# antonbaumann/MIMO-Unet

Measured on AMD Instinct MI355X. Metric: train images/sec at 256x256, S=2, fbc=30, higher is better.
Workload: dtype f32 (split into 16-bit hi/lo pairs on the MFMA; weight gradient: activation as one fp16 value); 1 GPU; cfg3: SEN12TP-shape synthetic 2->1 ch, 256x256, S=2, fbc=30, laplace_nll, batch 32 global; global_batch=32, per_gpu_batch=32, scaling=strong, labels=U[0,1) (SURVEY 8d); same batch every step, parallelism=dp1, world_size=1, weak_per_gpu_batch=32, strong_global_batch=32, optimizer=adam(lr=1e-3) fused, inputs=resident in HBM

## Files before the change

mimo_unet_amd/csrc/elementwise.hip:

```cpp
#include <hip/hip_ext.h>

#include <algorithm>
#include <cstdlib>

#include "elementwise.h"
#include "philox.h"

namespace mimo {

struct PQ {
  int q;
  int ql, pl;
  int QB, PPI;
  int p, pstep;
  bool active;
};

template <int T = 256>
__device__ __forceinline__ PQ pixquad(int Cv, bool xcd_bands = false) {
  PQ r;
  r.QB = Cv < T ? Cv : T;
  r.PPI = T / r.QB;
  r.ql = threadIdx.x % r.QB;
  r.pl = threadIdx.x / r.QB;
  r.q = blockIdx.y * r.QB + r.ql;
  r.active = r.pl < r.PPI && r.q < Cv;
  int bx = blockIdx.x;
  if (xcd_bands && (gridDim.x & 7) == 0) bx = (bx & 7) * (gridDim.x >> 3) + (bx >> 3);
  r.p = bx * r.PPI + r.pl;
  r.pstep = gridDim.x * r.PPI;
  return r;
}

constexpr int kBlocksBnRelu = 1536, kBlocksBnBwd = 1792, kBlocksUpBwd = 16384, kBlocksPoolBwd = 8192;
constexpr int kBnReduceThreads = 1024, kBlocksBnReduce = kBlocksBnBwd / 4;
static dim3 pq_grid(int Cv, int64_t P, int max_blocks = kEwMaxBlocks, int T = 256) {
  const int QB = Cv < T ? Cv : T;
  const int PPI = T / QB;
  int64_t gx = ceil_div64(P, PPI);
  if (gx > max_blocks) gx = max_blocks;
  if (gx < 1) gx = 1;
  return dim3((unsigned)gx, (unsigned)ceil_div(Cv, QB));
}

__device__ __forceinline__ float4 ld4(const float* p) { return *reinterpret_cast<const float4*>(p); }
__device__ __forceinline__ void st4(float* p, float4 v) { *reinterpret_cast<float4*>(p) = v; }
typedef __bf16 bf16x4_st __attribute__((ext_vector_type(4)));
typedef _Float16 f16x4_st __attribute__((ext_vector_type(4)));
__device__ __forceinline__ float4 ld4(const __bf16* p) {
  const bf16x4_st v = *reinterpret_cast<const bf16x4_st*>(p);
  return make_float4((float)v[0], (float)v[1], (float)v[2], (float)v[3]);
}
__device__ __forceinline__ void st4(__bf16* p, float4 v) {
  bf16x4_st r;
  r[0] = (__bf16)v.x;
  r[1] = (__bf16)v.y;
  r[2] = (__bf16)v.z;
  r[3] = (__bf16)v.w;
  *reinterpret_cast<bf16x4_st*>(p) = r;
}
__device__ __forceinline__ float4 ld4(const _Float16* p) {
  const f16x4_st v = *reinterpret_cast<const f16x4_st*>(p);
  return make_float4((float)v[0], (float)v[1], (float)v[2], (float)v[3]);
}
__device__ __forceinline__ void st4(_Float16* p, float4 v) {
  f16x4_st r;
  r[0] = (_Float16)v.x;
  r[1] = (_Float16)v.y;
  r[2] = (_Float16)v.z;
  r[3] = (_Float16)v.w;
  *reinterpret_cast<f16x4_st*>(p) = r;
}
#define MIMO_ST_DISPATCH(DT, T, ...) \
  switch (DT) {                      \
    case ST_BF16: {                  \
      typedef __bf16 T;              \
      __VA_ARGS__;                   \
    } break;                         \
    case ST_F16: {                   \
      typedef _Float16 T;            \
      __VA_ARGS__;                   \
    } break;                         \
    default: {                       \
      typedef float T;               \
      __VA_ARGS__;                   \
    } break;                         \
  }
#define MIMO_ST_DISPATCH2(DTZ, DTA, TZ, TA, ...) \
  if ((DTZ) == ST_F32) {                         \
    typedef float TZ;                            \
    MIMO_ST_DISPATCH(DTA, TA, __VA_ARGS__)       \
  } else if ((DTA) == ST_BF16) {                 \
    typedef __bf16 TZ;                           \
    typedef __bf16 TA;                           \
    __VA_ARGS__;                                 \
  } else {                                       \
    typedef _Float16 TZ;                         \
    typedef _Float16 TA;                         \
    __VA_ARGS__;                                 \
  }

__device__ __forceinline__ float4 f4add(float4 a, float4 b) { return make_float4(a.x + b.x, a.y + b.y, a.z + b.z, a.w + b.w); }
__device__ __forceinline__ float4 f4zero() { return make_float4(0.f, 0.f, 0.f, 0.f); }
__device__ __forceinline__ float4 f4max(float4 a, float4 b) {
  return make_float4(fmaxf(a.x, b.x), fmaxf(a.y, b.y), fmaxf(a.z, b.z), fmaxf(a.w, b.w));
}

__device__ __forceinline__ float4 quad_block_sum(float4 v, const PQ& t, float4* red) {
  __syncthreads();
  red[threadIdx.x] = t.active ? v : f4zero();
  __syncthreads();
  float4 s = f4zero();
  if (t.PPI <= 32) {
    if (t.pl == 0)
      for (int j = 0; j < t.PPI; ++j) s = f4add(s, red[j * t.QB + t.ql]);
    return s;
  }
  const bool lead = t.pl < 16 && t.pl < t.PPI;
  if (lead)
    for (int j = t.pl; j < t.PPI; j += 16) s = f4add(s, red[j * t.QB + t.ql]);
  __syncthreads();
  if (lead) red[threadIdx.x] = s;
  __syncthreads();
  s = f4zero();
  if (t.pl == 0)
    for (int j = 0; j < 16 && j < t.PPI; ++j) s = f4add(s, red[j * t.QB + t.ql]);
  return s;
}

template <typename T>
__device__ __forceinline__ float4 fold_read(const T* dxpad, int ldp, int n, int y, int x, int H, int W, int ch) {
  const T* base = dxpad + (size_t)n * (H + 2) * (W + 2) * ldp + ch;
  float4 s = ld4(base + ((size_t)(y + 1) * (W + 2) + (x + 1)) * ldp);
  const bool ya = y == 1, yb = y == H - 2, xa = x == 1, xb = x == W - 2;
  if (ya | yb | xa | xb) {
    const int ry[3] = {y, -1, H}, rx[3] = {x, -1, W};
    const bool vy[3] = {true, ya, yb}, vx[3] = {true, xa, xb};
#pragma unroll
    for (int i = 0; i < 3; ++i)
#pragma unroll
      for (int j = 0; j < 3; ++j)
        if (i + j > 0 && vy[i] && vx[j]) s = f4add(s, ld4(base + ((size_t)(ry[i] + 1) * (W + 2) + (rx[j] + 1)) * ldp));
  }
  return s;
}

struct PixIter {
  int n, y, x, dn, dy, dx;
};
__device__ __forceinline__ PixIter pix_iter(int p0, int pstep, int H, int W) {
  PixIter it;
  const int HW = H * W;
  it.n = p0 / HW;
  int r = p0 - it.n * HW;
  it.y = r / W;
  it.x = r - it.y * W;
  it.dn = pstep / HW;
  r = pstep - it.dn * HW;
// ... 879 lines not shown
          for (int j = 0; j < 6; ++j) {
            const float ww = ey[e] * (j < 4 ? wx[j] : ex[j - 4]);
            v.x += ww * g[j].x;
            v.y += ww * g[j].y;
            v.z += ww * g[j].z;
            v.w += ww * g[j].w;
          }
        }
        if (ex[e] != 0.f) {
          float4 g[4];
#pragma unroll
          for (int k = 0; k < 4; ++k) g[k] = ld4(base + ((size_t)(cy[k] + 1) * (W + 2) + prx[e]) * ldp);
#pragma unroll
          for (int k = 0; k < 4; ++k) {
            const float ww = wy[k] * ex[e];
            v.x += ww * g[k].x;
            v.y += ww * g[k].y;
            v.z += ww * g[k].z;
            v.w += ww * g[k].w;
          }
        }
      }
    }
    return v;
}

template <typename T>
__global__ void up_bwd_kernel(const T* __restrict__ dxpad, int ldp, int choff, T* __restrict__ da, int ldda,
                              int N, int H, int W, int h, int w, int padT, int padL, int Cv, int accumulate) {
  const PQ t = pixquad(Cv, true);
  if (!t.active) return;
  const int P = N * h * w;
  PixIter it = pix_iter(t.p, t.pstep, h, w);
  for (int p = t.p; p < P; p += t.pstep, pix_next(it, h, w)) {
    float4 v = up_bwd_pixel(dxpad, ldp, choff, t.q, it.n, it.y, it.x, H, W, h, w, padT, padL);
    T* dst = da + (size_t)p * ldda + 4 * t.q;
    if (accumulate) v = f4add(v, ld4(dst));
    st4(dst, v);
  }
}


int up_bwd_launch(const void* dxpad, int dt, int ldp, int choff, void* da, int ldda, int N, int H, int W, int h, int w,
                  int Cp, int accumulate, hipStream_t st) {
  const int Cv = Cp / 4;
  const int padT = (H - 2 * h) / 2, padL = (W - 2 * w) / 2;
  MIMO_ST_DISPATCH(dt, T, hipLaunchKernelGGL(up_bwd_kernel<T>, pq_grid(Cv, (int64_t)N * h * w, kBlocksUpBwd), dim3(256), 0, st,
                                             (const T*)dxpad, ldp, choff, (T*)da, ldda, N, H, W, h, w, padT, padL, Cv, accumulate));
  MIMO_KERNEL_CHECK();
  return MIMO_OK;
}

__device__ __forceinline__ float nll_value(int kind, float d, float lp, float eps_min, float eps_max) {
  const float sc = fminf(fmaxf(expf(lp), eps_min), eps_max);
  return kind == MIMO_LOSS_LAPLACE_NLL ? logf(sc) + fabsf(d) / sc : logf(sc) + d * d / sc;
}
__device__ __forceinline__ void nll_grad(int kind, float d, float lp, float eps_min, float eps_max, float* gmu, float* glp) {
  const float e = expf(lp);
  const float sc = fminf(fmaxf(e, eps_min), eps_max);
  if (kind == MIMO_LOSS_LAPLACE_NLL) {
    const float sgn = d > 0.f ? 1.f : (d < 0.f ? -1.f : 0.f);
    *gmu = sgn / sc;
    *glp = (1.f / sc - fabsf(d) / (sc * sc)) * e;
  } else {
    *gmu = 2.f * d / sc;
    *glp = (1.f / sc - d * d / (sc * sc)) * e;
  }
}

struct HeadLane {
  float4 w0, w1;
  float coef;
};
__device__ __forceinline__ HeadLane head_lane(const HeadGrad& h, int q, bool active) {
  HeadLane l;
  l.w0 = l.w1 = f4zero();
  l.coef = h.dloss ? h.dloss[h.s] * h.inv_count : 0.f;
  if (active) {
    const int c0 = 4 * q;
    float* a0 = reinterpret_cast<float*>(&l.w0);
    float* a1 = reinterpret_cast<float*>(&l.w1);
#pragma unroll
    for (int j = 0; j < 4; ++j) {
      a0[j] = c0 + j < h.C ? h.w[c0 + j] : 0.f;
      a1[j] = c0 + j < h.C ? h.w[h.C + c0 + j] : 0.f;
    }
  }
  return l;
}
__device__ __forceinline__ void head_dlogit(const HeadGrad& h, const HeadLane& l, int p, float* d0, float* d1) {
  const int n = p / h.HW;
  const int yx = p - n * h.HW;
  const int64_t obase = (((int64_t)n * h.S + h.s) * 2) * h.HW + yx;
  float a = h.dout ? h.dout[obase] : 0.f, b = h.dout ? h.dout[obase + h.HW] : 0.f;
  if (h.dloss) {
    const int64_t src = h.perm ? h.perm[(int64_t)h.s * h.N + n] : n;
    const float mk = h.mask ? h.mask[src * h.HW + yx] : 1.f;
    const float mu = h.out[obase], lp = h.out[obase + h.HW], y = h.label[src * h.HW + yx];
    float gm, gl;
    nll_grad(h.kind, mu - y, lp, h.eps_min, h.eps_max, &gm, &gl);
    a += l.coef * mk * gm;
    b += l.coef * mk * gl;
  }
  *d0 = a;
  *d1 = b;
}

__device__ __forceinline__ float4 relu_gate4(float4 g, float4 v, float4 sc, float4 sh) {
  g.x = fmaf(v.x, sc.x, sh.x) > 0.f ? g.x : 0.f;
  g.y = fmaf(v.y, sc.y, sh.y) > 0.f ? g.y : 0.f;
  g.z = fmaf(v.z, sc.z, sh.z) > 0.f ? g.z : 0.f;
  g.w = fmaf(v.w, sc.w, sh.w) > 0.f ? g.w : 0.f;
  return g;
}

template <typename TZ, typename TA>
__device__ __forceinline__ int pool_cell4(const GradSrc& s, const TZ* z, int ldz, int n, int cy, int cx, int H, int W, int q,
                                          float4 sc, float4 sh, bool masked, float4 m, float4 zz[4], float4 g[4]) {
  const int Hp = H / 2, Wp = W / 2, y0 = 2 * cy, x0 = 2 * cx;
  const bool win = cy < Hp && cx < Wp;
  const int valid = win ? 15 : ((1 | (x0 + 1 < W ? 2 : 0)) | (y0 + 1 < H ? (4 | (x0 + 1 < W ? 8 : 0)) : 0));
  const TZ* zs = z + (((size_t)n * H + y0) * W + x0) * ldz + 4 * q;
#pragma unroll
  for (int j = 0; j < 4; ++j) zz[j] = (valid >> j) & 1 ? ld4(zs + ((size_t)(j >> 1) * W + (j & 1)) * ldz) : f4zero();
  float4 gp = f4zero();
  if (win) gp = fold_read((const TA*)s.dxpad, s.ldp, n, cy, cx, Hp, Wp, s.choff + 4 * q);
#pragma unroll
  for (int j = 0; j < 4; ++j)
    g[j] = (s.skip && ((valid >> j) & 1)) ? fold_read((const TA*)s.skip, s.ldsk, n, y0 + (j >> 1), x0 + (j & 1), H, W, s.skoff + 4 * q)
                                           : f4zero();
  if (win) {
    auto act = [&](float v, float k, float b, float mm) { return fmaxf(fmaf(v, k, b), 0.f) * mm; };
#pragma unroll
    for (int j = 0; j < 4; ++j) {
      g[j].x = route_max(gp.x, act(zz[0].x, sc.x, sh.x, m.x), act(zz[1].x, sc.x, sh.x, m.x), act(zz[2].x, sc.x, sh.x, m.x), act(zz[3].x, sc.x, sh.x, m.x), j) + g[j].x;
      g[j].y = route_max(gp.y, act(zz[0].y, sc.y, sh.y, m.y), act(zz[1].y, sc.y, sh.y, m.y), act(zz[2].y, sc.y, sh.y, m.y), act(zz[3].y, sc.y, sh.y, m.y), j) + g[j].y;
      g[j].z = route_max(gp.z, act(zz[0].z, sc.z, sh.z, m.z), act(zz[1].z, sc.z, sh.z, m.z), act(zz[2].z, sc.z, sh.z, m.z), act(zz[3].z, sc.z, sh.z, m.z), j) + g[j].z;
      g[j].w = route_max(gp.w, act(zz[0].w, sc.w, sh.w, m.w), act(zz[1].w, sc.w, sh.w, m.w), act(zz[2].w, sc.w, sh.w, m.w), act(zz[3].w, sc.w, sh.w, m.w), j) + g[j].w;
    }
  }
#pragma unroll
  for (int j = 0; j < 4; ++j) {
    if (masked) {
      g[j].x *= m.x;
      g[j].y *= m.y;
      g[j].z *= m.z;
      g[j].w *= m.w;
    }
    g[j] = relu_gate4(g[j], zz[j], sc, sh);
  }
  return valid;
}

template <int SRC, typename TZ, typename TA>
__device__ __forceinline__ float4 relu_grad4(const GradSrc& s, const HeadLane& hl, const float* mask, int C, int p,
                                             const PixIter& it, int q, int H, int W, float4 v, float4 sc, float4 sh, float* d0,
                                             float* d1) {
  static_assert(SRC != GS_POOL, "pooled tensors: pool_cell4");
  float4 g;
  const int n = it.n;
  float4 m = make_float4(1.f, 1.f, 1.f, 1.f);
  if (mask) m = mask4(mask, n, C, 4 * q);
  if constexpr (SRC == GS_PLAIN) {
    g = ld4((const TA*)s.da + (size_t)p * s.ldda + 4 * q);
  } else if constexpr (SRC == GS_FOLD) {
    g = fold_read((const TA*)s.dxpad, s.ldp, n, it.y, it.x, H, W, 4 * q);
  } else {
    head_dlogit(s.head, hl, p, d0, d1);
    g = f4zero();
    g.x = fmaf(*d1, hl.w1.x, fmaf(*d0, hl.w0.x, g.x));
    g.y = fmaf(*d1, hl.w1.y, fmaf(*d0, hl.w0.y, g.y));
    g.z = fmaf(*d1, hl.w1.z, fmaf(*d0, hl.w0.z, g.z));
    g.w = fmaf(*d1, hl.w1.w, fmaf(*d0, hl.w0.w, g.w));
  }
  if (mask) {
    g.x *= m.x;
    g.y *= m.y;
    g.z *= m.z;
    g.w *= m.w;
  }
  return relu_gate4(g, v, sc, sh);
}

template <typename TZ, typename TA, int SRC>
__global__ __launch_bounds__(kBnReduceThreads) void bnrelu_bwd_reduce_kernel(
    const GradSrc src, const TZ* __restrict__ z, int ldz,
    const float* __restrict__ scale, const float* __restrict__ shift, const float* __restrict__ mean,
    const float* __restrict__ invstd, const float* __restrict__ mask, int C, int Cv, int N, int H, int W,
    float* __restrict__ partial) {
  __shared__ float4 red[kBnReduceThreads];
  const PQ t = pixquad<kBnReduceThreads>(Cv);
  const int Cp = 4 * Cv;
  float4 a1 = f4zero(), a2 = f4zero();
  float4 hw0 = f4zero(), hw1 = f4zero();
  float hb0 = 0.f, hb1 = 0.f;
  HeadLane hl = {};
  if constexpr (SRC == GS_HEAD) hl = head_lane(src.head, t.q, t.active);
  if (t.active) {
    const float4 sc = ld4(scale + 4 * t.q), sh = ld4(shift + 4 * t.q), mu = ld4(mean + 4 * t.q), is = ld4(invstd + 4 * t.q);
    if constexpr (SRC == GS_POOL) {
      const int Hc = (H + 1) / 2, Wc = (W + 1) / 2, P = N * Hc * Wc;
      PixIter it = pix_iter(t.p, t.pstep, Hc, Wc);
      for (int p = t.p; p < P; p += t.pstep, pix_next(it, Hc, Wc)) {
        float4 zz[4], g[4];
        const float4 m = mask ? mask4(mask, it.n, C, 4 * t.q) : make_float4(1.f, 1.f, 1.f, 1.f);
        const int valid = pool_cell4<TZ, TA>(src, z, ldz, it.n, it.y, it.x, H, W, t.q, sc, sh, mask != nullptr, m, zz, g);
#pragma unroll
        for (int j = 0; j < 4; ++j)
          if ((valid >> j) & 1) {
            a1 = f4add(a1, g[j]);
            a2.x += g[j].x * (zz[j].x - mu.x) * is.x;
            a2.y += g[j].y * (zz[j].y - mu.y) * is.y;
            a2.z += g[j].z * (zz[j].z - mu.z) * is.z;
            a2.w += g[j].w * (zz[j].w - mu.w) * is.w;
          }
      }
    } else {
      const int P = N * H * W;
      PixIter it = pix_iter(t.p, t.pstep, H, W);
      for (int p = t.p; p < P; p += t.pstep, pix_next(it, H, W)) {
        const float4 v = ld4(z + (size_t)p * ldz + 4 * t.q);
        float d0 = 0.f, d1 = 0.f;
        const float4 g = relu_grad4<SRC, TZ, TA>(src, hl, mask, C, p, it, t.q, H, W, v, sc, sh, &d0, &d1);
        a1 = f4add(a1, g);
        a2.x += g.x * (v.x - mu.x) * is.x;
        a2.y += g.y * (v.y - mu.y) * is.y;
        a2.z += g.z * (v.z - mu.z) * is.z;
        a2.w += g.w * (v.w - mu.w) * is.w;
        if constexpr (SRC == GS_HEAD) {
          const float4 av = bn_relu4(v, sc, sh);
          hw0.x = fmaf(d0, av.x, hw0.x);
          hw0.y = fmaf(d0, av.y, hw0.y);
          hw0.z = fmaf(d0, av.z, hw0.z);
          hw0.w = fmaf(d0, av.w, hw0.w);
          hw1.x = fmaf(d1, av.x, hw1.x);
          hw1.y = fmaf(d1, av.y, hw1.y);
          hw1.z = fmaf(d1, av.z, hw1.z);
          hw1.w = fmaf(d1, av.w, hw1.w);
          hb0 += d0;
          hb1 += d1;
        }
      }
    }
  }
  const float4 s1 = quad_block_sum(a1, t, red);
  const float4 s2 = quad_block_sum(a2, t, red);
  if (t.pl == 0 && t.q < Cv) {
    float* row = partial + (size_t)blockIdx.x * 2 * Cp;
    st4(row + 4 * t.q, s1);
    st4(row + Cp + 4 * t.q, s2);
  }
  if constexpr (SRC == GS_HEAD) {
    float* row = src.head.partial + (size_t)blockIdx.x * (2 * Cp + 2);
    const float4 w0 = quad_block_sum(hw0, t, red);
    const float4 w1 = quad_block_sum(hw1, t, red);
    const float4 sb = quad_block_sum(make_float4(hb0, hb1, 0.f, 0.f), t, red);
    if (t.pl == 0 && t.q < Cv) {
      st4(row + 4 * t.q, w0);
      st4(row + Cp + 4 * t.q, w1);
    }
    if (t.pl == 0 && t.q == 0) {
      row[2 * Cp] = sb.x;
      row[2 * Cp + 1] = sb.y;
    }
  }
}

static int check_grad_src(const GradSrc& src, int dta, int dtz) {
  if (src.kind < GS_PLAIN || src.kind > GS_HEAD || (src.kind >= GS_POOL && (dta != ST_F32 || dtz != ST_F32)) ||
      (src.kind == GS_HEAD && src.head.Co != 2)) {
    set_error("BatchNorm backward: gradient source %d unsupported here", src.kind);
    return MIMO_ERR_INVALID;
  }
  return MIMO_OK;
}

int bnrelu_bwd_reduce_launch(const GradSrc& src, int dta, const void* z, int dtz, int ldz,
                             const float* scale, const float* shift, const float* mean, const float* invstd,
                             const float* mask, int C, int Cp, int N, int H, int W, float* partial, int* rows,
                             hipStream_t st) {
  MIMO_TRY(check_grad_src(src, dta, dtz));
  const int Cv = Cp / 4;
  const int64_t units = src.kind == GS_POOL ? (int64_t)N * ((H + 1) / 2) * ((W + 1) / 2) : (int64_t)N * H * W;
  const dim3 grid = pq_grid(Cv, units, src.kind >= GS_POOL ? 256 : kBlocksBnReduce, kBnReduceThreads);
  *rows = grid.x;
#define REDUCE_LAUNCH(TZ, TA, SRC)                                                                                              \
  hipLaunchKernelGGL((bnrelu_bwd_reduce_kernel<TZ, TA, SRC>), grid, dim3(kBnReduceThreads), 0, st, src, (const TZ*)z, ldz, scale, \
                     shift, mean, invstd, mask, C, Cv, N, H, W, partial)
  if (src.kind == GS_POOL) {
    REDUCE_LAUNCH(float, float, GS_POOL);
  } else if (src.kind == GS_HEAD) {
    REDUCE_LAUNCH(float, float, GS_HEAD);
  } else if (src.kind == GS_PLAIN) {
    MIMO_ST_DISPATCH2(dtz, dta, TZ, TA, REDUCE_LAUNCH(TZ, TA, GS_PLAIN))
  } else {
    MIMO_ST_DISPATCH2(dtz, dta, TZ, TA, REDUCE_LAUNCH(TZ, TA, GS_FOLD))
  }
#undef REDUCE_LAUNCH
  MIMO_KERNEL_CHECK();
  return MIMO_OK;
}

__global__ __launch_bounds__(kColsumThreads) void bn_bwd_stats_kernel(const float* __restrict__ partial, int rows, int C,
                                                                      int Cp, double count, int training,
                                                                      float* __restrict__ c1, float* __restrict__ c2,
                                                                      float* __restrict__ dgamma, float* __restrict__ dbeta,
                                                                      float* __restrict__ dbias_zero, int* __restrict__ status) {
  __shared__ double red[2048];
  const int c = blockIdx.x * 64 + (threadIdx.x & 63);
  double s1, s2;
  grid_colsum2(partial, rows, (size_t)2 * Cp, c, Cp + c, c < Cp, true, red, &s1, &s2);
  if (c >= Cp || threadIdx.x >= 64) return;
  if (status && c < C && !(isfinite(s1) && isfinite(s2))) atomicOr(status, kStatusBwdStats);
  c1[c] = training ? (float)(s1 / count) : 0.f;
  c2[c] = training ? (float)(s2 / count) : 0.f;
  if (c < C) {
    if (dgamma) dgamma[c] = (float)s2;
    if (dbeta) dbeta[c] = (float)s1;
    if (dbias_zero) dbias_zero[c] = 0.f;
  }
}

int bn_bwd_stats_launch(const float* partial, int rows, int C, int Cp, int64_t count, int training, float* c1, float* c2,
                        float* dgamma, float* dbeta, float* dbias_zero, int* status, hipStream_t st) {
  hipLaunchKernelGGL(bn_bwd_stats_kernel, dim3(ceil_div(Cp, 64)), dim3(kColsumThreads), 0, st, partial, rows, C, Cp, (double)count,
                     training, c1, c2, dgamma, dbeta, dbias_zero, status);
  MIMO_KERNEL_CHECK();
  return MIMO_OK;
}

typedef __bf16 bf16x4_ew __attribute__((ext_vector_type(4)));
__device__ __forceinline__ void st_split4(float* base, size_t p, int Cp, int q, float4 r) {
  bf16x4_ew hi, lo;
  hi[0] = (__bf16)r.x;
  hi[1] = (__bf16)r.y;
  hi[2] = (__bf16)r.z;
  hi[3] = (__bf16)r.w;
  lo[0] = (__bf16)(r.x - (float)hi[0]);
  lo[1] = (__bf16)(r.y - (float)hi[1]);
  lo[2] = (__bf16)(r.z - (float)hi[2]);
  lo[3] = (__bf16)(r.w - (float)hi[3]);
  const int ch = 4 * q, chunk = ch >> 5, rc = min(32, Cp - 32 * chunk);
  unsigned char* d = reinterpret_cast<unsigned char*>(base) + p * (size_t)Cp * 4 + chunk * 128 + (ch & 31) * 2;
  *reinterpret_cast<bf16x4_ew*>(d) = hi;
  *reinterpret_cast<bf16x4_ew*>(d + 2 * rc) = lo;
}

__device__ __forceinline__ void block_absmax_store(float* slots, float v) {
  __shared__ float wm[16];
#pragma unroll
  for (int d = 1; d < 64; d <<= 1) v = fmaxf(v, __shfl_xor(v, d));
  if ((threadIdx.x & 63) == 0) wm[threadIdx.x >> 6] = v;
  __syncthreads();
  if (threadIdx.x == 0) {
    float m = wm[0];
    for (int i = 1; i < (int)(blockDim.x >> 6); ++i) m = fmaxf(m, wm[i]);
    slots[blockIdx.y * gridDim.x + blockIdx.x] = m;
  }
}
__device__ __forceinline__ float absmax4(float m, float4 r) {
  return fmaxf(fmaxf(m, fmaxf(fabsf(r.x), fabsf(r.y))), fmaxf(fabsf(r.z), fabsf(r.w)));
}

__global__ void split_pairs_kernel(const float* __restrict__ src, float* __restrict__ dst, int Cv, int64_t P,
                                   float* __restrict__ absmax) {
  const PQ t = pixquad(Cv);
  float amax = 0.f;
  if (t.active)
    for (int64_t p = t.p; p < P; p += t.pstep) {
      const float4 r = ld4(src + (size_t)p * 4 * Cv + 4 * t.q);
      st_split4(dst, (size_t)p, 4 * Cv, t.q, r);
      amax = absmax4(amax, r);
    }
  if (absmax) block_absmax_store(absmax, amax);
}

int split_pairs_launch(const float* src, float* dst, int64_t P, int Cp, hipStream_t st, float* absmax, int* absmax_n) {
  const dim3 grid = pq_grid(Cp / 4, P, 2048);
  if (absmax && (int)(grid.x * grid.y) > kDzMaxSlots) {
    set_error("split_pairs: %d x %d workgroups exceed the max |dz| slots", (int)grid.x, (int)grid.y);
    return MIMO_ERR_INVALID;
  }
  if (absmax_n) *absmax_n = (int)(grid.x * grid.y);
  hipLaunchKernelGGL(split_pairs_kernel, grid, dim3(256), 0, st, src, dst, Cp / 4, P, absmax);
  MIMO_KERNEL_CHECK();
  return MIMO_OK;
}

constexpr int kApplyMinWaves = 7;
template <typename TZ, typename TA, int SRC>
__global__ __launch_bounds__(256, (SRC == GS_PLAIN || SRC == GS_FOLD) ? kApplyMinWaves : 1) void bn_bwd_apply_kernel(const GradSrc src, const TZ* __restrict__ z, int ldz, const float* __restrict__ scale,
                                    const float* __restrict__ shift, const float* __restrict__ mean,
                                    const float* __restrict__ invstd, const float* __restrict__ mask, int C,
                                    const float* __restrict__ c1, const float* __restrict__ c2, int Cv, int N, int H,
                                    int W, TA* __restrict__ dz, int split_out, float* __restrict__ partial,
                                    float* __restrict__ absmax) {
  __shared__ float4 red[256];
  const PQ t = pixquad(Cv);
  const int Cp = 4 * Cv;
  float4 acc = f4zero();
  float amax = 0.f;
  HeadLane hl = {};
  if constexpr (SRC == GS_HEAD) hl = head_lane(src.head, t.q, t.active);
  if (t.active) {
    const float4 sc = ld4(scale + 4 * t.q), sh = ld4(shift + 4 * t.q), mu = ld4(mean + 4 * t.q), is = ld4(invstd + 4 * t.q);
    const float4 k1 = ld4(c1 + 4 * t.q), k2 = ld4(c2 + 4 * t.q);
    auto emit = [&](int p, float4 g, float4 v) {
      float4 r;
      r.x = sc.x * (g.x - k1.x - (v.x - mu.x) * is.x * k2.x);
      r.y = sc.y * (g.y - k1.y - (v.y - mu.y) * is.y * k2.y);
      r.z = sc.z * (g.z - k1.z - (v.z - mu.z) * is.z * k2.z);
      r.w = sc.w * (g.w - k1.w - (v.w - mu.w) * is.w * k2.w);
      if (split_out)
        st_split4(reinterpret_cast<float*>(dz), p, Cp, t.q, r);
      else
        st4(dz + (size_t)p * Cp + 4 * t.q, r);
      acc = f4add(acc, r);
      amax = absmax4(amax, r);
    };
    if constexpr (SRC == GS_POOL) {
      const int Hc = (H + 1) / 2, Wc = (W + 1) / 2, P = N * Hc * Wc;
      PixIter it = pix_iter(t.p, t.pstep, Hc, Wc);
      for (int p = t.p; p < P; p += t.pstep, pix_next(it, Hc, Wc)) {
        float4 zz[4], g[4];
        const float4 m = mask ? mask4(mask, it.n, C, 4 * t.q) : make_float4(1.f, 1.f, 1.f, 1.f);
        const int valid = pool_cell4<TZ, TA>(src, z, ldz, it.n, it.y, it.x, H, W, t.q, sc, sh, mask != nullptr, m, zz, g);
        const int p0 = (it.n * H + 2 * it.y) * W + 2 * it.x;
#pragma unroll
        for (int j = 0; j < 4; ++j)
          if ((valid >> j) & 1) emit(p0 + (j >> 1) * W + (j & 1), g[j], zz[j]);
      }
    } else {
      const int P = N * H * W;
      if (t.p < P) {
        const int p_last = t.p + (P - 1 - t.p) / t.pstep * t.pstep;
        PixIter it = pix_iter(p_last, t.pstep, H, W);
        for (int p = p_last; p >= 0; p -= t.pstep, pix_prev(it, H, W)) {
          const float4 v = ld4(z + (size_t)p * ldz + 4 * t.q);
          float d0, d1;
          emit(p, relu_grad4<SRC, TZ, TA>(src, hl, mask, C, p, it, t.q, H, W, v, sc, sh, &d0, &d1), v);
        }
      }
    }
  }
  if (absmax) block_absmax_store(absmax, amax);
  if (!partial) return;
  const float4 s = quad_block_sum(acc, t, red);
  if (t.pl == 0 && t.q < Cv) st4(partial + (size_t)blockIdx.x * Cp + 4 * t.q, s);
}

int bn_bwd_apply_launch(const GradSrc& src, int dta, const void* z, int dtz, int ldz,
                        const float* scale, const float* shift, const float* mean, const float* invstd, const float* mask,
                        int C, const float* c1, const float* c2, int Cp, int N, int H, int W, void* dz, int split_out,
                        float* partial, int* rows, hipStream_t st, float* absmax, int* absmax_n, hipEvent_t done) {
  MIMO_TRY(check_grad_src(src, dta, dtz));
  const int Cv = Cp / 4;
  const int64_t units = src.kind == GS_POOL ? (int64_t)N * ((H + 1) / 2) * ((W + 1) / 2) : (int64_t)N * H * W;
  const dim3 grid = pq_grid(Cv, units, src.kind == GS_POOL ? 1024 : src.kind == GS_HEAD ? 1280 : kBlocksBnBwd);
  *rows = grid.x;
  if (absmax_n) *absmax_n = (int)(grid.x * grid.y);
  if (absmax && (int)(grid.x * grid.y) > kDzMaxSlots) {
    set_error("bn_bwd_apply: %d x %d workgroups exceed the max |dz| slots", (int)grid.x, (int)grid.y);
    return MIMO_ERR_INVALID;
  }
  if (split_out && dta != ST_F32) {
    set_error("bn_bwd_apply: pair-split dz exists for fp32 storage only");
    return MIMO_ERR_INVALID;
  }
#define APPLY_LAUNCH(TZ, TA, SRC)                                                                                              \
  hipExtLaunchKernelGGL((bn_bwd_apply_kernel<TZ, TA, SRC>), grid, dim3(256), 0, st, nullptr, done, 0, src, (const TZ*)z, ldz, scale, \
                        shift, mean, invstd, mask, C, c1, c2, Cv, N, H, W, (TA*)dz, split_out, partial, absmax)
  if (src.kind == GS_POOL) {
    APPLY_LAUNCH(float, float, GS_POOL);
  } else if (src.kind == GS_HEAD) {
    APPLY_LAUNCH(float, float, GS_HEAD);
  } else if (src.kind == GS_PLAIN) {
    MIMO_ST_DISPATCH2(dtz, dta, TZ, TA, APPLY_LAUNCH(TZ, TA, GS_PLAIN))
  } else {
    MIMO_ST_DISPATCH2(dtz, dta, TZ, TA, APPLY_LAUNCH(TZ, TA, GS_FOLD))
  }
#undef APPLY_LAUNCH
  MIMO_KERNEL_CHECK();
  return MIMO_OK;
}

template <int G, int CO, typename T>
__global__ void head_fwd_kernel(const T* __restrict__ a, int lda, const float* __restrict__ w,
                                const float* __restrict__ bias, int C, int Cp, int Co, int N, int S, int s, int HW,
                                float* __restrict__ out, int* __restrict__ status, const float* __restrict__ in_scale,
                                const float* __restrict__ in_shift) {
  const int g = threadIdx.x % G, pl = threadIdx.x / G;
  constexpr int PPB = 256 / G, UN = 4;
  float wq[CO][4], bs[CO];
#pragma unroll
  for (int co = 0; co < CO; ++co) {
    bs[co] = co < Co ? bias[co] : 0.f;
#pragma unroll
    for (int j = 0; j < 4; ++j) wq[co][j] = (co < Co && 4 * g + j < C) ? w[co * C + 4 * g + j] : 0.f;
  }
  const bool has = 4 * g < Cp;
  const bool fin = in_scale != nullptr;
  const float4 isc = (fin && has) ? ld4(in_scale + 4 * g) : f4zero(), ish = (fin && has) ? ld4(in_shift + 4 * g) : f4zero();
  const int64_t P = (int64_t)N * HW, stride = (int64_t)gridDim.x * PPB;
  for (int64_t p0 = (int64_t)blockIdx.x * PPB + pl; p0 < P; p0 += stride * UN) {
    float4 v[UN];
#pragma unroll
    for (int u = 0; u < UN; ++u) {
      const int64_t p = p0 + u * stride;
      v[u] = (has && p < P) ? ld4(a + p * lda + 4 * g) : f4zero();
      if (fin) v[u] = bn_relu4(v[u], isc, ish);
    }
#pragma unroll
    for (int u = 0; u < UN; ++u) {
      const int64_t p = p0 + u * stride;
      float acc[CO];
#pragma unroll
      for (int co = 0; co < CO; ++co)
        acc[co] = fmaf(v[u].x, wq[co][0], fmaf(v[u].y, wq[co][1], fmaf(v[u].z, wq[co][2], v[u].w * wq[co][3])));
#pragma unroll
      for (int off = 1; off < G; off <<= 1)
#pragma unroll
        for (int co = 0; co < CO; ++co) acc[co] += __shfl_xor(acc[co], off);
      if (p < P) {
        const int n = (int)(p / HW);
        const int yx = (int)(p - (int64_t)n * HW);
#pragma unroll
        for (int co = 0; co < CO; ++co)
          if (co < Co && co % G == g) {
            const float o = acc[co] + bs[co];
            out[(((int64_t)n * S + s) * Co + co) * HW + yx] = o;
            if (status && !isfinite(o)) atomicOr(status, kStatusLogits);
          }
      }
    }
  }
}

int head_fwd_launch(const void* a, int dt, int lda, const float* w, const float* bias, int C, int Co, int N, int S, int s,
                    int HW, float* out, hipStream_t st, int* status, const float* in_scale, const float* in_shift) {
  if (Co > kMaxHeadOut || C > 256) {
    set_error("head: out_channels %d > %d or filter_base_count %d > 256 unsupported", Co, kMaxHeadOut, C);
    return MIMO_ERR_INVALID;
  }
  const int Cp = pad_channels(C), Cv = Cp / 4;
  int G = 2;
  while (G < Cv) G <<= 1;
  const int64_t P = (int64_t)N * HW;
  const int blocks = (int)std::min<int64_t>(ceil_div64(P, (256 / G) * 4), 4096);
#define HEAD_LAUNCH2(GG, CC)                                                                                         \
  MIMO_ST_DISPATCH(dt, T, hipLaunchKernelGGL((head_fwd_kernel<GG, CC, T>), dim3(blocks), dim3(256), 0, st, (const T*)a, lda, w, bias, \
                                             C, Cp, Co, N, S, s, HW, out, status, in_scale, in_shift))
#define HEAD_LAUNCH(GG)             \
  if (Co <= 2) {                    \
    HEAD_LAUNCH2(GG, 2);            \
  } else if (Co <= 4) {             \
    HEAD_LAUNCH2(GG, 4);            \
  } else {                          \
    HEAD_LAUNCH2(GG, kMaxHeadOut);  \
  }
  switch (G) {
    case 2: HEAD_LAUNCH(2); break;
    case 4: HEAD_LAUNCH(4); break;
    case 8: HEAD_LAUNCH(8); break;
    case 16: HEAD_LAUNCH(16); break;
    case 32: HEAD_LAUNCH(32); break;
    default: HEAD_LAUNCH(64); break;
  }
#undef HEAD_LAUNCH
#undef HEAD_LAUNCH2
  MIMO_KERNEL_CHECK();
  return MIMO_OK;
}

__global__ void loss_fwd_kernel(const float* __restrict__ out, const float* __restrict__ label,
                                const float* __restrict__ mask, const int64_t* __restrict__ perm, int N, int S, int Co,
                                int HW, int kind, float eps_min, float eps_max, float* __restrict__ partial) {
  __shared__ float red[256];
  const int s = blockIdx.y;
  const int Ct = Co / 2;
  const int64_t total = (int64_t)N * Ct * HW;
  float acc = 0.f;
  for (int64_t i = (int64_t)blockIdx.x * blockDim.x + threadIdx.x; i < total; i += (int64_t)gridDim.x * blockDim.x) {
    const int yx = (int)(i % HW);
    const int64_t r = i / HW;
    const int tch = (int)(r % Ct);
    const int n = (int)(r / Ct);
    const int64_t src = perm ? perm[(int64_t)s * N + n] : n;
    const float* o = out + (((int64_t)n * S + s) * Co) * HW + yx;
    const float mu = o[(int64_t)tch * HW], lp = o[(int64_t)(Ct + tch) * HW];
    const float y = label[(src * Ct + tch) * HW + yx];
    float v = nll_value(kind, mu - y, lp, eps_min, eps_max);
    if (mask) v *= mask[src * HW + yx];
    acc += v;
  }
  red[threadIdx.x] = acc;
  __syncthreads();
  for (int o = 128; o > 0; o >>= 1) {
    if ((int)threadIdx.x < o) red[threadIdx.x] += red[threadIdx.x + o];
    __syncthreads();
  }
  if (threadIdx.x == 0) partial[(size_t)s * gridDim.x + blockIdx.x] = red[0];
}

int loss_fwd_launch(const float* out, const float* label, const float* mask, const int64_t* perm, int N, int S, int Co,
                    int HW, int kind, float eps_min, float eps_max, float* partial, int* blocks, hipStream_t st) {
  const int64_t total = (int64_t)N * (Co / 2) * HW;
  const int nb = (int)std::min<int64_t>(ceil_div64(total, 256), 512);
  *blocks = nb;
  hipLaunchKernelGGL(loss_fwd_kernel, dim3(nb, S), dim3(256), 0, st, out, label, mask, perm, N, S, Co, HW, kind, eps_min,
                     eps_max, partial);
  MIMO_KERNEL_CHECK();
  return MIMO_OK;
}

__global__ void loss_finalize_kernel(const float* __restrict__ partial, int S, int blocks, double count,
// ... 185 lines not shown
```

Before: 1368 images/s.

## Restructure folded-gradient BN backward to iterate padded and off-ring pixels directly

The BatchNorm-ReLU backward reduce kernel now walks the padded gradient buffer linearly, two elements per step, gathering z through reflection, instead of calling fold_read once per output pixel. The apply kernel splits pixels into off-ring interior pixels, which take a single direct load, and ring pixels next to the reflection border, which still use fold_read. The aim is to drop the multi-tap gather of reflected-pad contributions from the common path. In exchange the code adds index helpers, size guards for small or huge inputs, and more complex iteration logic.

```diff
diff --git a/mimo_unet_amd/csrc/elementwise.hip b/mimo_unet_amd/csrc/elementwise.hip
--- a/mimo_unet_amd/csrc/elementwise.hip
+++ b/mimo_unet_amd/csrc/elementwise.hip
@@ -4,6 +4,7 @@
 #include <cstdlib>
 
 #include "elementwise.h"
+#include "fold_index.h"
 #include "philox.h"
 
 namespace mimo {
@@ -1189,19 +1190,30 @@
   return valid;
 }
 
+__device__ __forceinline__ float4 mask_gate4(float4 g, const float* mask, int n, int C, int q, float4 v, float4 sc, float4 sh) {
+  if (mask) {
+    const float4 m = mask4(mask, n, C, 4 * q);
+    g.x *= m.x;
+    g.y *= m.y;
+    g.z *= m.z;
+    g.w *= m.w;
+  }
+  return relu_gate4(g, v, sc, sh);
+}
+
+constexpr int kFoldUnroll = 2;
+
 template <int SRC, typename TZ, typename TA>
 __device__ __forceinline__ float4 relu_grad4(const GradSrc& s, const HeadLane& hl, const float* mask, int C, int p,
                                              const PixIter& it, int q, int H, int W, float4 v, float4 sc, float4 sh, float* d0,
                                              float* d1) {
-  static_assert(SRC != GS_POOL, "pooled tensors: pool_cell4");
+  static_assert(SRC != GS_POOL && SRC != GS_FOLD, "pooled tensors: pool_cell4; folded gradients: the kernels' own loops");
   float4 g;
   const int n = it.n;
   float4 m = make_float4(1.f, 1.f, 1.f, 1.f);
   if (mask) m = mask4(mask, n, C, 4 * q);
   if constexpr (SRC == GS_PLAIN) {
     g = ld4((const TA*)s.da + (size_t)p * s.ldda + 4 * q);
-  } else if constexpr (SRC == GS_FOLD) {
-    g = fold_read((const TA*)s.dxpad, s.ldp, n, it.y, it.x, H, W, 4 * q);
   } else {
     head_dlogit(s.head, hl, p, d0, d1);
     g = f4zero();
@@ -1220,7 +1232,7 @@
 }
 
 template <typename TZ, typename TA, int SRC>
-__global__ __launch_bounds__(kBnReduceThreads) void bnrelu_bwd_reduce_kernel(
+__global__ __launch_bounds__(kBnReduceThreads, SRC == GS_FOLD ? 8 : 1) void bnrelu_bwd_reduce_kernel(
     const GradSrc src, const TZ* __restrict__ z, int ldz,
     const float* __restrict__ scale, const float* __restrict__ shift, const float* __restrict__ mean,
     const float* __restrict__ invstd, const float* __restrict__ mask, int C, int Cv, int N, int H, int W,
@@ -1251,6 +1263,45 @@
             a2.z += g[j].z * (zz[j].z - mu.z) * is.z;
             a2.w += g[j].w * (zz[j].w - mu.w) * is.w;
           }
+      }
+    } else if constexpr (SRC == GS_FOLD) {
+      constexpr int U = kFoldUnroll;
+      const int Q = N * (H + 2) * (W + 2);
+      const TA* gsrc = (const TA*)src.dxpad + 4 * t.q;
+      const TZ* zsrc = z + 4 * t.q;
+      fold::PadIter it = fold::pad_iter(t.p, t.pstep, H, W);
+      for (int q = t.p; q < Q; q += U * t.pstep) {
+        float4 g[U], v[U];
+        bool ok[U];
+        int nn[U];
+        const fold::PadIter first = it;
+#pragma unroll
+        for (int j = 0; j < U; ++j) {
+          const int qj = q + j * t.pstep;
+          ok[j] = qj < Q;
+          fold::PadIter at = it;
+          at.n = ok[j] ? it.n : first.n;
+          at.y = ok[j] ? it.y : first.y;
+          at.x = ok[j] ? it.x : first.x;
+          g[j] = ld4(gsrc + (size_t)(ok[j] ? qj : q) * src.ldp);
+          v[j] = ld4(zsrc + (size_t)fold::pad_src_pixel(at, H, W) * ldz);
+          nn[j] = at.n;
+          fold::pad_next(it, H, W);
+        }
+#pragma unroll
+        for (int j = 0; j < U; ++j) {
+          float4 gj;
+          gj.x = ok[j] ? g[j].x : 0.f;
+          gj.y = ok[j] ? g[j].y : 0.f;
+          gj.z = ok[j] ? g[j].z : 0.f;
+          gj.w = ok[j] ? g[j].w : 0.f;
+          gj = mask_gate4(gj, mask, nn[j], C, t.q, v[j], sc, sh);
+          a1 = f4add(a1, gj);
+          a2.x += gj.x * (v[j].x - mu.x) * is.x;
+          a2.y += gj.y * (v[j].y - mu.y) * is.y;
+          a2.z += gj.z * (v[j].z - mu.z) * is.z;
+          a2.w += gj.w * (v[j].w - mu.w) * is.w;
+        }
       }
     } else {
       const int P = N * H * W;
@@ -1318,7 +1369,13 @@
                              hipStream_t st) {
   MIMO_TRY(check_grad_src(src, dta, dtz));
   const int Cv = Cp / 4;
-  const int64_t units = src.kind == GS_POOL ? (int64_t)N * ((H + 1) / 2) * ((W + 1) / 2) : (int64_t)N * H * W;
+  const int64_t units = src.kind == GS_POOL   ? (int64_t)N * ((H + 1) / 2) * ((W + 1) / 2)
+                        : src.kind == GS_FOLD ? (int64_t)N * (H + 2) * (W + 2)
+                                              : (int64_t)N * H * W;
+  if (src.kind == GS_FOLD && (H < 2 || W < 2 || units + (int64_t)kFoldUnroll * kBlocksBnReduce * kBnReduceThreads > INT32_MAX)) {
+    set_error("BatchNorm backward: folded source of %d x %d x %d pixels unsupported", N, H, W);
+    return MIMO_ERR_INVALID;
+  }
   const dim3 grid = pq_grid(Cv, units, src.kind >= GS_POOL ? 256 : kBlocksBnReduce, kBnReduceThreads);
   *rows = grid.x;
 #define REDUCE_LAUNCH(TZ, TA, SRC)                                                                                              \
@@ -1442,7 +1499,7 @@
   if (t.active) {
     const float4 sc = ld4(scale + 4 * t.q), sh = ld4(shift + 4 * t.q), mu = ld4(mean + 4 * t.q), is = ld4(invstd + 4 * t.q);
     const float4 k1 = ld4(c1 + 4 * t.q), k2 = ld4(c2 + 4 * t.q);
-    auto emit = [&](int p, float4 g, float4 v) {
+    auto emit = [&](size_t p, float4 g, float4 v) {
       float4 r;
       r.x = sc.x * (g.x - k1.x - (v.x - mu.x) * is.x * k2.x);
       r.y = sc.y * (g.y - k1.y - (v.y - mu.y) * is.y * k2.y);
@@ -1451,7 +1508,7 @@
       if (split_out)
         st_split4(reinterpret_cast<float*>(dz), p, Cp, t.q, r);
       else
-        st4(dz + (size_t)p * Cp + 4 * t.q, r);
+        st4(dz + p * Cp + 4 * t.q, r);
       acc = f4add(acc, r);
       amax = absmax4(amax, r);
     };
@@ -1466,6 +1523,33 @@
 #pragma unroll
         for (int j = 0; j < 4; ++j)
           if ((valid >> j) & 1) emit(p0 + (j >> 1) * W + (j & 1), g[j], zz[j]);
+      }
+    } else if constexpr (SRC == GS_FOLD) {
+      const TA* gsrc = (const TA*)src.dxpad;
+      const int c0 = 4 * t.q;
+      const int I = N * fold::off_ring_rows(H) * fold::off_ring_rows(W);
+      if (t.p < I) {
+        const int i_last = t.p + (I - 1 - t.p) / t.pstep * t.pstep;
+        fold::OffRingIter it = fold::off_ring_iter(i_last, t.pstep, H, W);
+        it.dn = __builtin_amdgcn_readfirstlane(it.dn);
+        it.dy = __builtin_amdgcn_readfirstlane(it.dy);
+        it.dx = __builtin_amdgcn_readfirstlane(it.dx);
+        for (int i = i_last; i >= 0; i -= t.pstep, fold::off_ring_prev(it, H, W)) {
+          const int y = fold::off_ring_line(it.jy, H), x = fold::off_ring_line(it.jx, W);
+          const int pp = (it.n * H + y) * W + x;
+          const size_t pq = ((size_t)it.n * (H + 2) + (y + 1)) * (W + 2) + (x + 1);
+          const float4 v = ld4(z + (size_t)pp * ldz + c0);
+          emit(pp, mask_gate4(ld4(gsrc + pq * src.ldp + c0), mask, it.n, C, t.q, v, sc, sh), v);
+        }
+      }
+      const int R = fold::ring_count(H, W), NR = N * R;
+      for (int r = t.p; r < NR; r += t.pstep) {
+        const int n = r / R;
+        int y, x;
+        fold::ring_pixel(r - n * R, H, W, &y, &x);
+        const size_t pp = ((size_t)n * H + y) * W + x;
+        const float4 v = ld4(z + pp * ldz + c0);
+        emit(pp, mask_gate4(fold_read((const TA*)src.dxpad, src.ldp, n, y, x, H, W, 4 * t.q), mask, n, C, t.q, v, sc, sh), v);
       }
     } else {
       const int P = N * H * W;
@@ -1498,6 +1582,10 @@
   if (absmax_n) *absmax_n = (int)(grid.x * grid.y);
   if (absmax && (int)(grid.x * grid.y) > kDzMaxSlots) {
     set_error("bn_bwd_apply: %d x %d workgroups exceed the max |dz| slots", (int)grid.x, (int)grid.y);
+    return MIMO_ERR_INVALID;
+  }
+  if (src.kind == GS_FOLD && (H < 2 || W < 2)) {
+    set_error("bn_bwd_apply: folded source of %d x %d pixels unsupported", H, W);
     return MIMO_ERR_INVALID;
   }
   if (split_out && dta != ST_F32) {
diff --git a/mimo_unet_amd/csrc/fold_index.h b/mimo_unet_amd/csrc/fold_index.h
--- /dev/null
+++ b/mimo_unet_amd/csrc/fold_index.h
@@ -0,0 +1,107 @@
+#pragma once
+
+#include <cstdint>
+
+#if defined(__HIPCC__)
+#define MIMO_FOLD_HD __host__ __device__ __forceinline__
+#else
+#define MIMO_FOLD_HD inline
+#endif
+
+namespace mimo {
+namespace fold {
+
+MIMO_FOLD_HD int iabs(int v) { return v < 0 ? -v : v; }
+MIMO_FOLD_HD int imin(int a, int b) { return a < b ? a : b; }
+MIMO_FOLD_HD int imax(int a, int b) { return a > b ? a : b; }
+
+MIMO_FOLD_HD int reflect_src(int y, int H) { return (H - 1) - iabs((H - 1) - iabs(y)); }
+
+struct PadIter {
+  int n, y, x, dn, dy, dx;
+};
+MIMO_FOLD_HD PadIter pad_iter(int q0, int qstep, int H, int W) {
+  PadIter it;
+  const int Wp = W + 2, HWp = (H + 2) * Wp;
+  it.n = q0 / HWp;
+  int r = q0 - it.n * HWp;
+  it.y = r / Wp;
+  it.x = r - it.y * Wp;
+  it.dn = qstep / HWp;
+  r = qstep - it.dn * HWp;
+  it.dy = r / Wp;
+  it.dx = r - it.dy * Wp;
+  return it;
+}
+MIMO_FOLD_HD void pad_next(PadIter& it, int H, int W) {
+  it.x += it.dx;
+  it.y += it.dy;
+  it.n += it.dn;
+  const int cx = it.x >= W + 2;
+  it.x -= cx ? W + 2 : 0;
+  it.y += cx;
+  const int cy = it.y >= H + 2;
+  it.y -= cy ? H + 2 : 0;
+  it.n += cy;
+}
+MIMO_FOLD_HD int64_t pad_src_pixel(const PadIter& it, int H, int W) {
+  return ((int64_t)it.n * H + reflect_src(it.y - 1, H)) * W + reflect_src(it.x - 1, W);
+}
+
+MIMO_FOLD_HD int ring_lines(int H) { return H == 3 ? 1 : 2; }
+MIMO_FOLD_HD bool on_ring(int y, int x, int H, int W) { return (y == 1) | (y == H - 2) | (x == 1) | (x == W - 2); }
+MIMO_FOLD_HD int off_ring_line(int j, int H) {
+  const int a = imin(1, H - 2), b = imax(1, H - 2);
+  const int y = j + (j >= a);
+  return y + ((b != a) & (y >= b));
+}
+MIMO_FOLD_HD int ring_count(int H, int W) { return ring_lines(H) * W + ring_lines(W) * (H - ring_lines(H)); }
+MIMO_FOLD_HD int off_ring_rows(int H) { return H - ring_lines(H); }
+MIMO_FOLD_HD void ring_pixel(int k, int H, int W, int* y, int* x) {
+  const int ny = ring_lines(H), nx = ring_lines(W);
+  const int rows = ny * W;
+  if (k < rows) {
+    const int i = k / W;
+    *y = i == 0 ? imin(1, H - 2) : imax(1, H - 2);
+    *x = k - i * W;
+  } else {
+    const int k2 = k - rows, j = k2 / nx, c = k2 - j * nx;
+    *y = off_ring_line(j, H);
+    *x = c == 0 ? imin(1, W - 2) : imax(1, W - 2);
+  }
+}
+
+struct OffRingIter {
+  int n, jy, jx, dn, dy, dx;
+};
+MIMO_FOLD_HD OffRingIter off_ring_iter(int i0, int istep, int H, int W) {
+  OffRingIter it;
+  const int Wi = off_ring_rows(W), HWi = off_ring_rows(H) * Wi;
+  it.n = i0 / HWi;
+  int r = i0 - it.n * HWi;
+  it.jy = r / Wi;
+  it.jx = r - it.jy * Wi;
+  it.dn = istep / HWi;
+  r = istep - it.dn * HWi;
+  it.dy = r / Wi;
+  it.dx = r - it.dy * Wi;
+  return it;
+}
+MIMO_FOLD_HD void off_ring_prev(OffRingIter& it, int H, int W) {
+  const int Hi = off_ring_rows(H), Wi = off_ring_rows(W);
+  it.jx -= it.dx;
+  it.jy -= it.dy;
+  it.n -= it.dn;
+  const int bx = it.jx < 0;
+  it.jx += bx ? Wi : 0;
+  it.jy -= bx;
+  const int by = it.jy < 0;
+  it.jy += by ? Hi : 0;
+  it.n -= by;
+}
+MIMO_FOLD_HD int64_t off_ring_pixel(const OffRingIter& it, int H, int W) {
+  return ((int64_t)it.n * H + off_ring_line(it.jy, H)) * W + off_ring_line(it.jx, W);
+}
+
+}
+}
```

After: 1378 images/s (median of 6 runs). No clear change (+0.7%).
